# quziyan/NPairLoss

Measured on NVIDIA H100. Metric: N-pair fwd+bwd samples/sec at B=8192,D=512, higher is better.
Workload: dtype f32 (3-pass fp16-split wgmma, f32 accumulate)

## Files before the change

### npairloss_b200/csrc/ctx.cu

```cuda
#include <cuda.h>
#include <cuda_bf16.h>
#include <cuda_fp16.h>
#include <cuda_runtime.h>
#include <sched.h>
#include <cudaTypedefs.h>
#include <dlfcn.h>

#include <cstdarg>
#include <cstdio>
#include <cstdlib>
#include <cmath>
#include <cstring>
#include <map>
#include <memory>
#include <mutex>
#include <string>
#include <vector>

#include "../../include/npair_b200.h"
#include "gemm_wgmma.cuh"
#include "grad_fused.cuh"
#include "host.cuh"
#include "kernels.cuh"

// ... 436 lines not shown
  if (c->ev_made) for (int i = 0; i < NPAIR_PROF_PHASES; ++i) { cudaEventDestroy(c->ev[i][0]); cudaEventDestroy(c->ev[i][1]); }
  delete c;
}

static int create_impl(const npair_config* cfg, const void* id128, void* ext_comm, npair_ctx** out);
static bool mma_is_symmetric(int prec, int device) {
  static std::mutex mu;
  static std::map<std::pair<int, int>, bool> cache;
  std::lock_guard<std::mutex> lk(mu);
  const std::pair<int, int> key(device, prec);
  auto it = cache.find(key);
  if (it != cache.end()) return it->second;
  bool ok = false;
  const int Q = 192, D = 96;
  npair_config cfg;
  npair_config_default(&cfg, Q, D);
  cfg.sim_precision = prec; cfg.device = device; cfg.flags = NPAIR_INTERNAL_FULL_TILES; cfg.num_tops = 2;
  npair_ctx* t = nullptr;
  if (create_impl(&cfg, nullptr, nullptr, &t) == NPAIR_OK) {
    std::vector<float> x(static_cast<size_t>(Q) * D), lab(Q), S(static_cast<size_t>(Q) * t->ldS);
    uint32_t rng = 12345u;
    for (int r = 0; r < Q; ++r) {
      double nrm = 0.0;
      for (int d = 0; d < D; ++d) { rng = rng * 1664525u + 1013904223u; const float v = static_cast<float>(static_cast<int32_t>(rng >> 8) % 2001 - 1000) * 1e-3f; x[static_cast<size_t>(r) * D + d] = v; nrm += static_cast<double>(v) * v; }
      const float inv = static_cast<float>(1.0 / sqrt(nrm > 0 ? nrm : 1.0));
      for (int d = 0; d < D; ++d) x[static_cast<size_t>(r) * D + d] *= inv;
      lab[r] = static_cast<float>(r / 2);
    }
    float *dx = nullptr, *dl = nullptr;
    float tops[5];
    if (cudaMalloc(&dx, sizeof(float) * x.size()) == cudaSuccess && cudaMalloc(&dl, sizeof(float) * Q) == cudaSuccess &&
        cudaMemcpy(dx, x.data(), sizeof(float) * x.size(), cudaMemcpyHostToDevice) == cudaSuccess &&
        cudaMemcpy(dl, lab.data(), sizeof(float) * Q, cudaMemcpyHostToDevice) == cudaSuccess &&
        npair_forward(t, dx, dl, tops, nullptr) == NPAIR_OK && cudaDeviceSynchronize() == cudaSuccess &&
        cudaMemcpy(S.data(), t->S, sizeof(float) * S.size(), cudaMemcpyDeviceToHost) == cudaSuccess) {
      ok = true;
      for (int i = 0; i < Q && ok; ++i)
        for (int j = 0; j < i; ++j)
          if (memcmp(&S[static_cast<size_t>(i) * t->ldS + j], &S[static_cast<size_t>(j) * t->ldS + i], 4) != 0) { ok = false; break; }
    }
    cudaFree(dx); cudaFree(dl);
    npair_destroy(t);
  }
  cudaGetLastError();
  cache[key] = ok;
  return ok;
}

static int create_impl(const npair_config* cfg, const void* id128, void* ext_comm, npair_ctx** out) {
  if (!out) { g_create_err = "null out"; return NPAIR_E_ARG; }
  *out = nullptr;
  std::string e;
  int rc = validate(cfg, &e);
  if (rc != NPAIR_OK) { g_create_err = e; return rc; }
  int device = -1, sms = 0;
  if ((rc = open_device(cfg->device, &device, &sms)) != NPAIR_OK) return rc;
  std::unique_ptr<npair_ctx, void (*)(npair_ctx*)> made(new npair_ctx(), npair_destroy);
  npair_ctx* c = made.get();
  c->cfg = *cfg; c->device = device; c->sms = sms;
  const bool blocks = sim_block_rows(*cfg) > 0;
  const bool ask_sym = (cfg->world > 1 && cfg->bwd_exchange == NPAIR_BWD_AUTO && cfg->gemm_backend == NPAIR_GEMM_TCGEN05) || blocks;
  const bool sym = !ask_sym || mma_is_symmetric(cfg->sim_precision, c->device);
  if (blocks && !sym) {
    g_create_err = "row-block similarity mode: the similarity GEMM is not bitwise symmetric on this device, so a recomputed block of S "
                   "would not match the rows the statistics were taken from";
    return NPAIR_E_ARG;
  }
  static_cast<Plan&>(*c) = plan_of(*cfg, c->sms, sym);
  c->Q = cfg->Q; c->D = cfg->D; c->world = cfg->world; c->rank = cfg->rank; c->prec = cfg->sim_precision;
  const int Q = c->Q, D = c->D, N = c->N, ns = c->nsplit;
  CREATE_TRY(ctx_buffers(c, c->mem));
  if (c->sym_tiles) {
    const std::vector<int2> tl = sym_tile_list(Q, N);
    CREATE_TRY(cudaMemcpy(c->sym_tiles, tl.data(), sizeof(int2) * tl.size(), cudaMemcpyHostToDevice));
  }
  CREATE_TRY(cudaHostAlloc(&c->tops_pinned, sizeof(TopsBlock), cudaHostAllocMapped));
  memset(c->tops_pinned, 0, sizeof(TopsBlock));
  CREATE_TRY(cudaHostGetDevicePointer(&c->tops_dev, c->tops_pinned, 0));
  CREATE_TRY(c->order.create());
  if (c->lsel_mask) CREATE_TRY(allow_local_select_smem());
  if (cfg->gemm_backend == NPAIR_GEMM_TCGEN05) {
    CREATE_TRY(allow_smem(gemm_kernel(c->prec, c->sweep_epi)));
    if (c->n_blocks > 1) CREATE_TRY(allow_smem(gemm_kernel(c->prec, EPI_STORE_S)));
    CREATE_TRY(c->fused_grad ? allow_smem(fused_kernel(c->prec)) : allow_smem(gemm_kernel(c->prec, EPI_OUT)));
    std::string te;
    const int bkg = c->bk_grad;
    const uint16_t* catA = c->cat ? c->XcatA : c->Xs;
    const uint16_t* catB = c->cat ? c->XcatB : c->Xs;
    bool ok = make_tmap_kcat(&c->tm_simA, &c->tm_simB, catA +static_cast<long long>(c->rank) * Q * c->kcat, Q, catB, N, c->kcat, &te);
    ok = ok && make_tmap_f32_store(&c->tm_S, c->S, N, c->s_rows, c->ldS, &te);
    if (c->H) ok = ok && make_tmap_pieces(&c->tm_b1A, c->H, N, Q, ns, c->Np, static_cast<long long>(Q) * c->Np, bkg, 128, &te);
    ok = ok && make_tmap_pieces(&c->tm_b1B, c->XsT, N, D, ns, c->Np, static_cast<long long>(D) * c->Np, bkg, 256, &te);
    if (c->fused_grad) {
      ok = ok && make_tmap_pieces(&c->tm_fB, c->XsT, N, D, ns, c->Np, static_cast<long long>(D) * c->Np, 32, 256, &te);
      ok = ok && make_tmap_f32_store(&c->tm_fS, c->S, N, c->s_rows, c->ldS, &te, 128);
    }
    if (c->bwd_mode == NPAIR_BWDMODE_REDUCE_SCATTER) {
      ok = ok && make_tmap_pieces(&c->tm_b2A, c->HT, Q, N, ns, c->Qp, static_cast<long long>(N) * c->Qp, bkg, 128, &te);
      ok = ok && make_tmap_pieces(&c->tm_b2B, c->XlT, Q, D, ns, c->Qp, static_cast<long long>(D) * c->Qp, bkg, 256, &te);
    }
    if (!ok) { g_create_err = te; return NPAIR_E_CUDA; }
  }
  if (c->world > 1 && (id128 || ext_comm)) {
    NcclApi* api = nccl_api();
    if (!api->h || !api->err.empty()) { g_create_err = api->err; return NPAIR_E_NCCL; }
    if (ext_comm) { c->comm = ext_comm; c->own_comm = false; }
    else {
      std::string ce;
      if (acquire_comm(id128, c->world, c->rank, &c->comm, &ce) != 0) { g_create_err = ce; c->comm = nullptr; return NPAIR_E_NCCL; }
      c->own_comm = true;
    }
  }
  if (c->comm && (c->want_p2p_feat || c->want_p2p_rec) && !getenv("NPAIR_NO_P2P")) {
    NcclApi* api = nccl_api();
    const int W = c->world;
    CREATE_TRY(p2p_buffers(c, c->mem));
    cudaIpcMemHandle_t mine;
    static_assert(sizeof(cudaIpcMemHandle_t) == 64, "IPC handle size");
    CREATE_TRY(cudaIpcGetMemHandle(&mine, c->p2p_region));
    char* d_all = nullptr;
    CREATE_TRY(cudaMalloc(&d_all, 64ull * (W + 1)));
    const std::unique_ptr<char, cudaError_t (*)(void*)> free_handles(d_all, cudaFree);
    char* d_mine = d_all + 64ull * W;
    CREATE_TRY(cudaMemcpy(d_mine, &mine, 64, cudaMemcpyHostToDevice));
    CREATE_TRY(cudaDeviceSynchronize());
    int r = api->AllGather(d_mine, d_all, 16, NCCL_FLOAT32, c->comm, nullptr);
    if (r != 0) { g_create_err = fmt("ncclAllGather(ipc handles): %s", api->GetErrorString(r)); return NPAIR_E_NCCL; }
    CREATE_TRY(cudaStreamSynchronize(nullptr));
    std::vector<cudaIpcMemHandle_t> all(W);
    CREATE_TRY(cudaMemcpy(all.data(), d_all, 64ull * W, cudaMemcpyDeviceToHost));
    std::vector<float*> pb(W);
    bool mapped = true;
    for (int q = 0; q < W && mapped; ++q) {
      if (q == c->rank) { pb[q] = c->p2p_region; continue; }
      void* a = nullptr;
      if (cudaIpcOpenMemHandle(&a, all[q], cudaIpcMemLazyEnablePeerAccess) != cudaSuccess) { cudaGetLastError(); mapped = false; break; }
      c->p2p_opened.push_back(a);
      pb[q] = static_cast<float*>(a);
    }
    if (mapped) {
      CREATE_TRY(cudaMemcpy(c->p2p_peer_base, pb.data(), sizeof(float*) * W, cudaMemcpyHostToDevice));
      c->p2p_feat = c->want_p2p_feat; c->p2p_rec = c->want_p2p_rec;
    }
  }
  if (c->wscope && !c->comm) {
    g_create_err = "global_scope with world > 1 needs a communicator (the world-scope reductions are internal)"; return NPAIR_E_ARG;
  }
  *out = made.release();
  return NPAIR_OK;
}

int npair_create(const npair_config* cfg, const void* id128, npair_ctx** out) { return create_impl(cfg, id128, nullptr, out); }
int npair_create_with_comm(const npair_config* cfg, void* comm, npair_ctx** out) {
  if (cfg && cfg->world > 1 && !comm) { g_create_err = "null communicator"; return NPAIR_E_ARG; }
  return create_impl(cfg, nullptr, comm, out);
}

static void p2p_push(npair_ctx* c, int kind, uint32_t ep, int blocks, const float* srcA, long long nA, int partA,
                     const float* srcB, long long nB, int partB, cudaStream_t st) {
  const long long par = ep & 1u;
  p2p_push_kernel<<<blocks, 256, 0, st>>>(srcA, nA, c->xl.off(partA, par, c->rank), srcB, nB, srcB ? c->xl.off(partB, par, c->rank) : 0,
                                          c->p2p_peer_base, c->xl.flags, xchg_flag(kind, par, c->world, c->rank), c->world, ep, c->p2p_ticket);
  count_launch();
}
static const float* p2p_wait(npair_ctx* c, int kind, uint32_t ep, int part, cudaStream_t st) {
  const long long par = ep & 1u;
  p2p_wait_kernel<<<1, 32, 0, st>>>(reinterpret_cast<const uint32_t*>(c->p2p_region + c->xl.flags) + xchg_flag(kind, par, c->world, 0), c->world, ep);
// ... 247 lines not shown
  if (!c) return NPAIR_E_ARG;
  if (!d_feat || !d_label || !d_diff || !tops_host) { c->err = "null pointer argument"; return NPAIR_E_ARG; }
  int rc;
  if ((rc = check_out_aligned(c, d_diff, "the gradient pointer")) != NPAIR_OK) return rc;
  if ((rc = need_comm(c, "npair_forward_gathered")) != NPAIR_OK) return rc;
  OrderedCall call(c, stream);
  if ((rc = call.enter()) != NPAIR_OK) return rc;
  if ((rc = forward_rank(c, d_feat, d_label, call.st)) != NPAIR_OK) return rc;
  if ((rc = backward_impl(c, loss_weight, d_diff, nullptr, nullptr, call.st)) != NPAIR_OK) return rc;
  return finish_forward(c, tops_host, call.st);
}

int npair_backward_partial(npair_ctx* c, float loss_weight, float* d_local_half, float* d_total_half, void* stream) {
  if (!c) return NPAIR_E_ARG;
  if (!d_local_half || (c->world > 1 && !d_total_half)) { c->err = "null gradient pointer"; return NPAIR_E_ARG; }
  int rc;
  if ((rc = check_out_aligned(c, d_local_half, "d_local_half")) != NPAIR_OK) return rc;
  if (c->world > 1 && (rc = check_out_aligned(c, d_total_half, "d_total_half")) != NPAIR_OK) return rc;
  if ((rc = need_forward(c, "npair_backward_partial")) != NPAIR_OK) return rc;
  if (c->bwd_mode == NPAIR_BWDMODE_ROW_SCALARS) { c->err = "this context exchanges row scalars: use npair_row_scalars + npair_backward_gathered"; return NPAIR_E_STATE; }
  OrderedCall call(c, stream);
  if ((rc = call.enter()) != NPAIR_OK) return rc;
  return backward_impl(c, loss_weight, d_local_half, c->world > 1 ? d_total_half : nullptr, nullptr, call.st);
}

int npair_row_scalars(npair_ctx* c, float* d_out, void* stream) {
  if (!c || !d_out) return NPAIR_E_ARG;
  int rc;
  if ((rc = need_forward(c, "npair_row_scalars")) != NPAIR_OK) return rc;
  OrderedCall call(c, stream);
  if ((rc = call.enter()) != NPAIR_OK) return rc;
  CUDA_TRY(c, cudaMemcpyAsync(d_out, c->ra.rowrec, sizeof(RowRecord) * c->Q, cudaMemcpyDeviceToDevice, call.st));
  return NPAIR_OK;
}

int npair_backward_gathered(npair_ctx* c, float loss_weight, const float* d_rs_total, float* d_diff, void* stream) {
  if (!c) return NPAIR_E_ARG;
  if (!d_rs_total || !d_diff) { c->err = "null pointer argument"; return NPAIR_E_ARG; }
  int rc;
  if ((rc = check_out_aligned(c, d_diff, "the gradient pointer")) != NPAIR_OK) return rc;
  if ((rc = need_forward(c, "npair_backward_gathered")) != NPAIR_OK) return rc;
  if (c->bwd_mode != NPAIR_BWDMODE_ROW_SCALARS) { c->err = "this context does not exchange row scalars (see npair_bwd_exchange_mode)"; return NPAIR_E_STATE; }
  OrderedCall call(c, stream);
  if ((rc = call.enter()) != NPAIR_OK) return rc;
  return backward_impl(c, loss_weight, d_diff, nullptr, reinterpret_cast<const RowRecord*>(d_rs_total), call.st);
}

static void reduce_splits(npair_ctx* c, int splits, int rows, float* d_diff, float beta, cudaStream_t st) {
  const long long n = split_part(1, rows, c->D);
  splitk_reduce_kernel<<<grid_for(n / 4, 8 * c->sms), 256, 0, st>>>(c->part, splits, n, d_diff, beta);
  count_launch();
}

static int backward_core(npair_ctx* c, float loss_weight, float* d_diff, float* d_total_ext, const RowRecord* d_rs_ext, cudaStream_t st) {
  const int Q = c->Q, N = c->N, D = c->D;
  const MiningParams mp = mining_of(c->cfg);
  const float lw_over_q = loss_weight / static_cast<float>(c->wscope ? N : Q);
  const bool tc = c->cfg.gemm_backend == NPAIR_GEMM_TCGEN05;
  const RowRecord* rs_total = nullptr;
  int bw_mode = BW_SYM;
  if (c->bwd_mode == NPAIR_BWDMODE_ROW_SCALARS) {
    bw_mode = BW_ROWSCAL;
    if (d_rs_ext) rs_total = d_rs_ext;
    else {
      if (c->p2p_rec && !c->step.ext_gathered) {
        PhaseTimer pt(c, 8, st);
        rs_total = reinterpret_cast<const RowRecord*>(p2p_wait(c, XCHG_RECORDS, c->p2p_rec_epoch, XP_REC, st));
      } else if (!c->step.rec_gathered) {
        PhaseTimer pt(c, 8, st);
        NcclApi* api = nccl_api();
        int r = api->AllGather(c->ra.rowrec, c->rs_total, ROW_RECORD_FLOATS * Q, NCCL_FLOAT32, c->comm, st);
        if (r != 0) { c->err = fmt("ncclAllGather(row records): %s", api->GetErrorString(r)); return NPAIR_E_NCCL; }
        c->step.rec_gathered = true;
        rs_total = c->rs_total;
      } else rs_total = c->rs_total;
    }
  } else if (c->bwd_mode == NPAIR_BWDMODE_REDUCE_SCATTER) bw_mode = BW_SPLIT;
  if (tc && c->fused_grad) {
    FusedGradParams fp; memset(&fp, 0, sizeof(fp));
    fp.N = N; fp.D = D;
    fp.colrec = rs_total ? rs_total : c->ra.rowrec;
    fp.inv_world = c->wscope ? 1.f : 1.f / static_cast<float>(c->world);
    fp.log2_world = c->wscope ? 0.f : log2f(static_cast<float>(c->world));
    fp.sgn_p = ap_sign(mp.ap_method); fp.sgn_n = an_sign(mp.an_method);
    fp.ldo = D; fp.alpha = 0.5f * lw_over_q; fp.beta = 0.f; fp.dev_scale = &c->bs->x_inv_scale;
    fp.part = c->part;
    fp.chunk_kb = c->grad_chunk_kb;
    PhaseTimer pt(c, 6, st);
    const int first = c->s_block_row0 >= 0 ? c->s_block_row0 / c->s_rows : 0;
    for (int k = 0; k < c->n_blocks; ++k) {
      const int r0 = (first + k) % c->n_blocks * c->s_rows, rows = Q - r0 < c->s_rows ? Q - r0 : c->s_rows;
      CUDA_TRY(c, recompute_sim_block(c, r0, st));
      const SimRows sim = sim_rows(c, r0, rows);
      fp.Q = sim.rows; fp.ts = tile_sched(sim.rows, D, c->grad_kblocks, c->grad_split); fp.m_blk0 = sim.row0 / TileShape::BM;
      fp.rowrec = c->ra.rowrec + sim.row0; fp.self_offset = sim.self_col(sim.row0); fp.out = d_diff + static_cast<long long>(sim.row0) * D;
      CUDA_TRY(c, launch_fused_grad(c->prec, c->tm_fB, c->tm_fS, fp, c->sms, st));
      if (fp.ts.splits > 1) reduce_splits(c, fp.ts.splits, rows, fp.out, 0.f, st);
    }
    CUDA_TRY(c, cudaGetLastError());
    return NPAIR_OK;
  }
  {
    PhaseTimer pt(c, 5, st);
    launch_build_weights(sim_rows(c, 0, Q), c->world, bw_mode, rs_total, mp, c->ra, c->prec, c->H, c->Np, c->HT, c->Qp, st);
  }
  GemmParams gp; memset(&gp, 0, sizeof(gp));
  gp.dev_scale = &c->bs->x_inv_scale;
  const bool rs_path = c->bwd_mode == NPAIR_BWDMODE_REDUCE_SCATTER;
  if (rs_path) {
    gp.M = N; gp.Nn = D; gp.ts = tile_sched(N, D, (Q + c->bk_grad - 1) / c->bk_grad);
    gp.out = d_total_ext ? d_total_ext : c->OUT2; gp.ldo = D; gp.alpha = 0.5f * (1.f / static_cast<float>(c->world)) * lw_over_q; gp.beta = 0.f;
    {
      PhaseTimer pt(c, 7, st);
      if (tc) CUDA_TRY(c, launch_gemm(c->prec, EPI_OUT,c->tm_b2A, c->tm_b2B, c->tm_S, gp, c->sms, st));
      else CUDA_TRY(c, launch_simt_gemm(c->prec, EPI_OUT, c->HT, c->Qp, static_cast<long long>(N) * c->Qp, c->XlT, c->Qp, static_cast<long long>(D) * c->Qp, Q, gp, st));
    }
    if (!d_total_ext) {
      PhaseTimer pt(c, 8, st);
      NcclApi* api = nccl_api();
      int r = api->ReduceScatter(c->OUT2, d_diff, static_cast<size_t>(Q) * D, NCCL_FLOAT32, NCCL_SUM, c->comm, st);
      if (r != 0) { c->err = fmt("ncclReduceScatter: %s", api->GetErrorString(r)); return NPAIR_E_NCCL; }
    }
  }
  gp.M = Q; gp.Nn = D; gp.ts = tile_sched(Q, D, c->grad_kblocks, c->grad_split);
  gp.out = d_diff; gp.ldo = D; gp.alpha = 0.5f * lw_over_q; gp.beta = (rs_path && !d_total_ext) ? 1.f : 0.f;
  gp.part = c->part;
  {
    PhaseTimer pt(c, 6, st);
    if (tc) CUDA_TRY(c, launch_gemm(c->prec, EPI_OUT,c->tm_b1A, c->tm_b1B, c->tm_S, gp, c->sms, st));
    else CUDA_TRY(c, launch_simt_gemm(c->prec, EPI_OUT, c->H, c->Np, static_cast<long long>(Q) * c->Np, c->XsT, c->Np, static_cast<long long>(D) * c->Np, N, gp, st));
    if (gp.ts.splits > 1) reduce_splits(c, gp.ts.splits, Q, d_diff, gp.beta, st);
  }
  CUDA_TRY(c, cudaGetLastError());
  return NPAIR_OK;
}

int npair_profile_enable(npair_ctx* c, int on) {
  if (!c) return NPAIR_E_ARG;
  CUDA_TRY(c, cudaSetDevice(c->device));
  if (on && !c->ev_made) {
    for (int i = 0; i < NPAIR_PROF_PHASES; ++i) { CUDA_TRY(c, cudaEventCreate(&c->ev[i][0])); CUDA_TRY(c, cudaEventCreate(&c->ev[i][1])); }
    c->ev_made = true;
  }
  c->prof = on != 0;
  for (int i = 0; i < NPAIR_PROF_PHASES; ++i) c->ev_used[i] = false;
  return NPAIR_OK;
}
unsigned long long npair_kernel_launches(void) { return npair::g_kernel_launches; }

static int await_calls(npair_ctx* c) {
  CUDA_TRY(c, cudaSetDevice(c->device));
  CUDA_TRY(c, cudaEventSynchronize(c->order.done));
  return NPAIR_OK;
}

int npair_profile_read(npair_ctx* c, float* ms_out) {
  if (!c || !ms_out) return NPAIR_E_ARG;
  const int rc = await_calls(c);
  if (rc != NPAIR_OK) return rc;
  for (int i = 0; i < NPAIR_PROF_PHASES; ++i) {
    ms_out[i] = 0.f;
    if (c->ev_made && c->ev_used[i]) { float ms = 0.f; CUDA_TRY(c, cudaEventElapsedTime(&ms, c->ev[i][0], c->ev[i][1])); ms_out[i] = ms; }
    c->ev_used[i] = false;
  }
  return NPAIR_OK;
}

__global__ void decode_ord_kernel(const uint32_t* __restrict__ in, float* __restrict__ out, int n) {
  const int i = blockIdx.x * blockDim.x + threadIdx.x;
  if (i < n) out[i] = ord2f(in[i]);
}
__global__ void int_to_float_kernel(const int* __restrict__ in, float* __restrict__ out, int n) {
  const int i = blockIdx.x * blockDim.x + threadIdx.x;
  if (i < n) out[i] = static_cast<float>(in[i]);
}

int npair_debug_read(npair_ctx* c, int which, float* dst, size_t n) {
  if (!c || !dst) return NPAIR_E_ARG;
  const int rc = await_calls(c);
// ... 131 lines not shown
```

### npairloss_b200/csrc/gemm.cu

```cuda
#include <cuda_bf16.h>
#include <cuda_fp16.h>
#include <cuda_runtime.h>

#include "gemm_wgmma.cuh"
#include "grad_fused.cuh"
#include "host.cuh"
#include "kernels.cuh"

namespace npair {

static int gemm_grid(const TileSched& ts, int sms) { return ts.num_tiles() < sms ? ts.num_tiles() : sms; }

template <int NSPLIT, bool BF16, int EPI, int BK>
static GemmKernel gemm_t() {
  using Cfg = GemmCfg<NSPLIT, BK, EPI>;
  return GemmKernel{split_gemm_kernel<NSPLIT, BF16, EPI, BK>, Cfg::THREADS, Cfg::SMEM_BYTES};
}
template <bool BF16>
static GemmKernel sim_gemm_t(int epi) {
  switch (epi) {
    case EPI_STORE_S | EPI_STATS: return gemm_t<1, BF16, EPI_STORE_S | EPI_STATS, 64>();
    case EPI_STORE_S | EPI_STATS | EPI_SYM: return gemm_t<1, BF16, EPI_STORE_S | EPI_STATS | EPI_SYM, 64>();
    case EPI_STATS: return gemm_t<1, BF16, EPI_STATS, 64>();
    case EPI_STATS | EPI_SYM: return gemm_t<1, BF16, EPI_STATS | EPI_SYM, 64>();
    case EPI_STORE_S: return gemm_t<1, BF16, EPI_STORE_S, 64>();
    case EPI_COUNT: return gemm_t<1, BF16, EPI_COUNT, 64>();
    case EPI_COUNT | EPI_SYM: return gemm_t<1, BF16, EPI_COUNT | EPI_SYM, 64>();
    case EPI_GATHER: return gemm_t<1, BF16, EPI_GATHER, 64>();
    case EPI_GATHER | EPI_SYM: return gemm_t<1, BF16, EPI_GATHER | EPI_SYM, 64>();
    case EPI_BUCKET: return gemm_t<1, BF16, EPI_BUCKET, 64>();
    case EPI_BUCKET | EPI_SYM: return gemm_t<1, BF16, EPI_BUCKET | EPI_SYM, 64>();
    case EPI_ARGMAX: return gemm_t<1, BF16, EPI_ARGMAX, 64>();
    default: return GemmKernel{nullptr, 0, 0};
  }
}
GemmKernel gemm_kernel(int prec, int epi) {
  return with_prec(prec, [epi](auto P) {
    constexpr SplitFormat f = SPLIT_FORMATS[P];
    return epi != EPI_OUT ? sim_gemm_t<f.bf16>(epi) : gemm_t<f.pieces, f.bf16, EPI_OUT, bk_of(P, EPI_OUT)>();
  });
}
cudaError_t launch_gemm(int prec, int epi, const CUtensorMap& a, const CUtensorMap& b, const CUtensorMap& sm, const GemmParams& p, int sms, cudaStream_t st) {
  const GemmKernel k = gemm_kernel(prec, epi);
  if (!k.fn) return cudaErrorInvalidValue;
  k.fn<<<gemm_grid(p.ts, sms), k.threads, k.smem, st>>>(a, b, sm, p);
  count_launch();
  return cudaGetLastError();
}

FusedKernel fused_kernel(int prec) {
  return with_prec(prec, [](auto P) {
    constexpr SplitFormat f = SPLIT_FORMATS[P];
    return FusedKernel{fused_grad_kernel<f.pieces, f.bf16>, FusedCfg<f.pieces>::THREADS, FusedCfg<f.pieces>::SMEM_BYTES};
  });
}
cudaError_t launch_fused_grad(int prec, const CUtensorMap& b, const CUtensorMap& sm, const FusedGradParams& p, int sms, cudaStream_t st) {
  const FusedKernel k = fused_kernel(prec);
  k.fn<<<gemm_grid(p.ts, sms), k.threads, k.smem, st>>>(b, sm, p);
  count_launch();
  return cudaGetLastError();
}

template <int PREC>
__device__ __forceinline__ float piece_sum(const uint16_t* base, long long off, long long ps) {
  if (PREC == PREC_BF16) return __bfloat162float(__ushort_as_bfloat16(base[off]));
  if (PREC == PREC_FP16X2) return __half2float(__ushort_as_half(base[off])) + __half2float(__ushort_as_half(base[ps + off]));
  return __bfloat162float(__ushort_as_bfloat16(base[off])) + __bfloat162float(__ushort_as_bfloat16(base[ps + off])) +
         __bfloat162float(__ushort_as_bfloat16(base[2 * ps + off]));
}
template <int PREC, int OUT>
__global__ void __launch_bounds__(256) simt_gemm_kernel(const uint16_t* __restrict__ A, long long lda, long long psA,
                                                        const uint16_t* __restrict__ B, long long ldb, long long psB, int K, GemmParams p) {
  __shared__ float As[16][65], Bs[16][65];
  const int tx = threadIdx.x & 15, ty = threadIdx.x >> 4;
  const int m0 = blockIdx.y * 64, n0 = blockIdx.x * 64;
  float acc[4][4] = {};
  for (int k0 = 0; k0 < K; k0 += 16) {
    for (int e = threadIdx.x; e < 64 * 16; e += 256) {
      const int r = e >> 4, kk = e & 15;
      const int gm = m0 + r, gn = n0 + r, gk = k0 + kk;
      As[kk][r] = (gm < p.M && gk < K) ? piece_sum<PREC>(A, static_cast<long long>(gm) * lda + gk, psA) : 0.f;
      Bs[kk][r] = (gn < p.Nn && gk < K) ? piece_sum<PREC>(B, static_cast<long long>(gn) * ldb + gk, psB) : 0.f;
    }
    __syncthreads();
#pragma unroll
    for (int kk = 0; kk < 16; ++kk) {
      float a[4], b[4];
#pragma unroll
      for (int i = 0; i < 4; ++i) { a[i] = As[kk][ty * 4 + i]; b[i] = Bs[kk][tx * 4 + i]; }
#pragma unroll
      for (int i = 0; i < 4; ++i)
#pragma unroll
        for (int j = 0; j < 4; ++j) acc[i][j] = fmaf(a[i], b[j], acc[i][j]);
    }
    __syncthreads();
  }
  const float inv = p.dev_scale ? *p.dev_scale : 1.f;
  for (int i = 0; i < 4; ++i) {
    const int row = m0 + ty * 4 + i;
    if (row >= p.M) continue;
    for (int j = 0; j < 4; ++j) {
      const int col = n0 + tx * 4 + j;
      if (col >= p.Nn) continue;
      if (!OUT) p.S[static_cast<long long>(row) * p.ldS + col] = acc[i][j] * inv * inv;
      else {
        float* d = p.out + static_cast<long long>(row) * p.ldo + col;
        float o = p.alpha * inv * acc[i][j];
        if (p.beta != 0.f) o += p.beta * *d;
        *d = o;
      }
    }
  }
}
cudaError_t launch_simt_gemm(int prec, int epi, const uint16_t* A, long long lda, long long psA, const uint16_t* B, long long ldb,
                             long long psB, int K, const GemmParams& p, cudaStream_t st) {
  dim3 grid((p.Nn + 63) / 64, (p.M + 63) / 64);
  with_prec(prec, [&](auto P) {
    auto kernel = epi == EPI_OUT ? simt_gemm_kernel<P, 1> : simt_gemm_kernel<P, 0>;
    kernel<<<grid, 256, 0, st>>>(A, lda, psA, B, ldb, psB, K, p);
  });
  count_launch();
  return cudaGetLastError();
}

__global__ void splitk_reduce_kernel(const float* __restrict__ part, int splits, long long n, float* __restrict__ out, float beta) {
  const long long t0 = static_cast<long long>(blockIdx.x) * blockDim.x + threadIdx.x, nth = static_cast<long long>(gridDim.x) * blockDim.x;
  const bool vec = (n & 3) == 0 && ((reinterpret_cast<uintptr_t>(part) | reinterpret_cast<uintptr_t>(out)) & 15) == 0;
  if (vec) {
    for (long long i = t0 * 4; i < n; i += nth * 4) {
      float4 a = *reinterpret_cast<const float4*>(part + i);
      for (int s = 1; s < splits; ++s) { const float4 b = *reinterpret_cast<const float4*>(part + s * n + i); a.x += b.x; a.y += b.y; a.z += b.z; a.w += b.w; }
      if (beta != 0.f) { const float4 o = *reinterpret_cast<const float4*>(out + i); a.x += beta * o.x; a.y += beta * o.y; a.z += beta * o.z; a.w += beta * o.w; }
      *reinterpret_cast<float4*>(out + i) = a;
    }
  } else {
    for (long long i = t0; i < n; i += nth) {
      float a = part[i];
      for (int s = 1; s < splits; ++s) a += part[s * n + i];
      if (beta != 0.f) a += beta * out[i];
      out[i] = a;
// ... 6 lines not shown
```

### npairloss_b200/csrc/grad_fused.cuh

```cuda
#pragma once
#include <cuda.h>
#include <cuda_bf16.h>
#include <cuda_fp16.h>
#include <cuda_runtime.h>
#include <stdint.h>

#include "gemm_wgmma.cuh"
#include "ptx.cuh"

namespace npair {

struct FusedGradParams {
  int Q, N, D;
  TileSched ts;
  int chunk_kb;
  float* part;
  const float* S;
  const RowRecord* rowrec;
  const RowRecord* colrec;
  int self_offset;
  float inv_world, log2_world;
  float sgn_p, sgn_n;
  float* out; long long ldo;
  float alpha, beta;
  const float* dev_scale;
  int m_blk0;
};

template <int NSPLIT>
struct FusedCfg {
  static constexpr int BM = 128, BN = 256, BK = 32;
  static constexpr int B_PIECE = BN * 64;
  static constexpr int S_TILE = BM * 128;
  static constexpr int CREC = BK * sizeof(RowRecord);
  static constexpr int STAGE_BYTES = NSPLIT * B_PIECE + S_TILE + CREC;
  static constexpr int NPASS = mma_passes(NSPLIT);
  static constexpr int STAGES_FIT = (227 * 1024 - 2048) / STAGE_BYTES;
  static constexpr int STAGES = STAGES_FIT > 6 ? 6 : STAGES_FIT;
  static constexpr int SMEM_BYTES = STAGES * STAGE_BYTES + 1024  + 1024 ;
  static constexpr int THREADS = 384;
};

template <int NSPLIT, bool BF16>
__device__ __forceinline__ void split_pair(float a, float b, uint32_t (&out)[3]) {
  if (NSPLIT == 1) {
    out[0] = static_cast<uint32_t>(__bfloat16_as_ushort(__float2bfloat16_rn(a))) | (static_cast<uint32_t>(__bfloat16_as_ushort(__float2bfloat16_rn(b))) << 16);
  } else if (NSPLIT == 2) {
    const __half2 h = __floats2half2_rn(a, b);
    const float2 hf = __half22float2(h);
    const __half2 l = __floats2half2_rn(a - hf.x, b - hf.y);
    out[0] = *reinterpret_cast<const uint32_t*>(&h);
    out[1] = *reinterpret_cast<const uint32_t*>(&l);
  } else {
    const __nv_bfloat162 h = __floats2bfloat162_rn(a, b);
    const float2 hf = __bfloat1622float2(h);
    const float r1a = a - hf.x, r1b = b - hf.y;
    const __nv_bfloat162 m = __floats2bfloat162_rn(r1a, r1b);
    const float2 mf = __bfloat1622float2(m);
    const __nv_bfloat162 l = __floats2bfloat162_rn(r1a - mf.x, r1b - mf.y);
    out[0] = *reinterpret_cast<const uint32_t*>(&h);
    out[1] = *reinterpret_cast<const uint32_t*>(&m);
    out[2] = *reinterpret_cast<const uint32_t*>(&l);
  }
}

__device__ __forceinline__ void red_add_v2(float* dst, float a, float b) {
  asm volatile("red.global.add.v2.f32 [%0], {%1, %2};" ::"l"(dst), "f"(a), "f"(b) : "memory");
}
__device__ __forceinline__ void red_add_f32(float* dst, float a) {
  asm volatile("red.global.add.f32 [%0], %1;" ::"l"(dst), "f"(a) : "memory");
}

__device__ __forceinline__ void bulk_copy_g2s(void* smem_dst, const void* gsrc, uint32_t bytes, uint64_t* bar) {
  asm volatile("cp.async.bulk.shared::cluster.global.mbarrier::complete_tx::bytes [%0], [%1], %2, [%3];"
               ::"r"(ptx::smem_u32(smem_dst)), "l"(reinterpret_cast<uint64_t>(gsrc)), "r"(bytes), "r"(ptx::smem_u32(bar))
               : "memory");
}

__device__ __forceinline__ int chunk_end(int c0, int kb0, int kb1, int ch, int key) {
  if (ch <= 0) return kb1;
  if (c0 == kb0) { const int first = max(1, (((key & 7) + 1) * ch) >> 3); return min(kb1, kb0 + first); }
  return min(kb1, c0 + ch);
}

struct RowRec { float m2r, tn, m2, lab, tp, cA; int self_col; };

__device__ __forceinline__ float select_f32(bool c, float a, float b) {
  float r;
  asm("{\n\t.reg .pred q;\n\tsetp.ne.b32 q, %3, 0;\n\tselp.f32 %0, %1, %2, q;\n\t}" : "=f"(r) : "f"(a), "f"(b), "r"(static_cast<int>(c)));
  return r;
}
__device__ __forceinline__ float pair_weight(float s, const RowRecord& c, const RowRec& r, int m, const FusedGradParams& p) {
  const bool same = !(c.label() != r.lab);
  const float kn = s * p.sgn_n;
  const float a1 = select_f32(same, fmaf(s, LOG2E, -r.m2), select_f32(kn <= r.tn, fmaf(s, LOG2E, -r.m2r), -INFINITY));
  const float a2 = select_f32(same, fmaf(s, LOG2E, -c.m2()), select_f32(kn <= c.thr_n(), fmaf(s, LOG2E, -c.m2c()), -INFINITY));
  float e1, e2;
  asm("ex2.approx.ftz.f32 %0, %1;" : "=f"(e1) : "f"(a1));
  asm("ex2.approx.ftz.f32 %0, %1;" : "=f"(e2) : "f"(a2));
  const float kp = s * p.sgn_p;
  const float w1 = select_f32(kp <= r.tp, e1 * r.cA, 0.f);
  const float w2 = select_f32(kp <= c.thr_p(), e2 * c.cA(), 0.f);
  const float g = select_f32(same, fmaf(w2, p.inv_world, w1), e1 + e2);
  return (m == r.self_col || m >= p.N) ? 0.f : g;
}

__device__ __forceinline__ RowRec load_rowrec(const FusedGradParams& p, int row) {
  RowRec r;
  r.m2 = 0.f; r.m2r = INFINITY; r.tp = -INFINITY; r.tn = -INFINITY; r.cA = 0.f; r.lab = 0.f;
  r.self_col = row + p.self_offset;
  if (row < p.Q) {
    const RowRecord c = p.rowrec[row];
    r.m2r = c.m2c() - p.log2_world; r.tn = c.thr_n(); r.m2 = c.m2(); r.lab = c.label(); r.tp = c.thr_p(); r.cA = c.cA();
  }
  return r;
}

template <int NSPLIT, bool BF16>
__global__ void __launch_bounds__(384, 1)
fused_grad_kernel(const __grid_constant__ CUtensorMap tmapB, const __grid_constant__ CUtensorMap tmapS, const FusedGradParams p) {
  using Cfg = FusedCfg<NSPLIT>;
  const int worker = static_cast<int>(blockIdx.x), num_workers = static_cast<int>(gridDim.x);
  constexpr int BM = Cfg::BM, BN = Cfg::BN, BK = Cfg::BK, STAGES = Cfg::STAGES;
  extern __shared__ uint8_t smem_raw[];
  uint8_t* smem = smem_raw + ((1024u - (ptx::smem_u32(smem_raw) & 1023u)) & 1023u);
  StageRing<STAGES> ring(smem + STAGES * Cfg::STAGE_BYTES);

  const int warp = threadIdx.x >> 5, lane = threadIdx.x & 31;
  const int num_tiles = p.ts.num_tiles();
  const float inv_scale = p.dev_scale ? *p.dev_scale : 1.f;
  const float alpha = p.alpha * inv_scale;

  if (warp == 8 && lane == 0) {
    ptx::prefetch_tmap(&tmapB); ptx::prefetch_tmap(&tmapS);
    ring.init();
  }
  __syncthreads();

  if (warp >= 8) {
    asm volatile("setmaxnreg.dec.sync.aligned.u32 40;");
    if (warp == 8 && lane == 0) {
      for (int tile = worker; tile < num_tiles; tile += num_workers) {
        const Tile t = p.ts.at(tile);
        for (int kb = t.kb0; kb < t.kb1; ++kb) {
          const int m0 = kb * BK;
          const uint32_t crec_bytes = static_cast<uint32_t>(min(BK, p.N - m0)) * static_cast<uint32_t>(sizeof(RowRecord));
          uint64_t* full = ring.produce(NSPLIT * Cfg::B_PIECE + Cfg::S_TILE + crec_bytes);
          uint8_t* st = smem + ring.stage * Cfg::STAGE_BYTES;
#pragma unroll
          for (int s = 0; s < NSPLIT; ++s)
            ptx::tma_load_3d(st + s * Cfg::B_PIECE, &tmapB, full, m0, t.n_blk * BN, s);
          ptx::tma_load_2d(st + NSPLIT * Cfg::B_PIECE, &tmapS, full, m0, t.m_blk * BM);
          bulk_copy_g2s(st + NSPLIT * Cfg::B_PIECE + Cfg::S_TILE, p.colrec + m0, crec_bytes, full);
          ring.advance();
        }
      }
    }
  } else {
    asm volatile("setmaxnreg.inc.sync.aligned.u32 232;");
    constexpr int KSTEPS = BK / 16;
    static_assert(KSTEPS % 2 == 0, "a K block's first step must use A buffer 0");
    const int g = warp >> 2, wi = warp & 3;
    const int c4 = lane & 3;
    const int rl0 = g * 64 + wi * 16 + (lane >> 2);
    auto build = [&](uint32_t (&af)[NSPLIT][4], const RowRec (&rr)[2], int st_idx, int kb, int k2) {
      const uint8_t* s_tile = smem + st_idx * Cfg::STAGE_BYTES + NSPLIT * Cfg::B_PIECE;
      const RowRecord* crec = reinterpret_cast<const RowRecord*>(s_tile + Cfg::S_TILE);
#pragma unroll
      for (int t = 0; t < 2; ++t) {
        const int k = 16 * k2 + 8 * t + 2 * c4;
        const int m = kb * BK + k;
        const RowRecord c0 = RowRecord::load(crec, k), c1 = RowRecord::load(crec, k + 1);
#pragma unroll
        for (int h = 0; h < 2; ++h) {
          const int rl = rl0 + 8 * h;
          const float2 s2 = *reinterpret_cast<const float2*>(s_tile + rl * 128 + (((k >> 2) ^ (rl & 7)) << 4) + (k & 3) * 4);
          const float w0 = pair_weight(s2.x, c0, rr[h], m, p);
          const float w1 = pair_weight(s2.y, c1, rr[h], m + 1, p);
          uint32_t o[3];
          split_pair<NSPLIT, BF16>(w0, w1, o);
#pragma unroll
          for (int s = 0; s < NSPLIT; ++s) af[s][2 * t + h] = o[s];
        }
      }
    };
    for (int tile = worker; tile < num_tiles; tile += num_workers) {
      const Tile t = p.ts.at(tile);
      const int ckey = ((p.m_blk0 + t.m_blk) >> 1) + t.n_blk + t.split;
      float* obase = p.ts.splits > 1 ? p.part + split_part(t.split, p.Q, p.ldo) : p.out;
      const float beta = p.ts.splits > 1 ? 0.f : p.beta;
      RowRec rr[2];
#pragma unroll
      for (int h = 0; h < 2; ++h) rr[h] = load_rowrec(p, t.m_blk * BM + rl0 + 8 * h);
      float acc[128];
      uint32_t af[2][NSPLIT][4];
      for (int c0 = t.kb0, c1; c0 < t.kb1; c0 = c1) {
        c1 = chunk_end(c0, t.kb0, t.kb1, p.chunk_kb, ckey);
        ring.wait_full();
        build(af[0], rr, ring.stage, c0, 0);
        int prev = ring.stage;
        for (int kb = c0; kb < c1; ++kb) {
          const int cur = ring.stage;
          const uint32_t b0 = ptx::smem_u32(smem + cur * Cfg::STAGE_BYTES);
          ring.advance();
#pragma unroll
          for (int k2 = 0; k2 < KSTEPS; ++k2) {
            ptx::wgmma_fence();
#pragma unroll
            for (int ps = 0; ps < Cfg::NPASS; ++ps) {
              int sa, sb;
              pass_pieces(NSPLIT, ps, sa, sb);
              const uint64_t bd = ptx::make_kmajor_desc(b0 + sb * Cfg::B_PIECE + k2 * 32, 512u, 2u);
              ptx::wgmma_m64n256k16_rs<BF16>(acc, af[k2 & 1][sa], bd, ((kb - c0) | ps | k2) != 0 ? 1u : 0u);
            }
            ptx::wgmma_commit();
            ptx::wgmma_wait<1>();
            if (k2 == 0 && kb != c0) ring.release(prev, lane);
            if (k2 + 1 < KSTEPS) {
              build(af[(k2 + 1) & 1], rr, cur, kb, k2 + 1);
            } else if (kb + 1 < c1) {
              ring.wait_full();
              build(af[0], rr, ring.stage, kb + 1, 0);
            }
          }
          prev = cur;
        }
        ptx::wgmma_wait<0>();
        ptx::fence_regs(acc);
        ring.release(prev, lane);
        const bool first = (c0 == t.kb0);
#pragma unroll
        for (int j = 0; j < 32; ++j) {
          const int col = t.n_blk * BN + 8 * j + 2 * c4;
#pragma unroll
          for (int h = 0; h < 2; ++h) {
            const int row = t.m_blk * BM + rl0 + 8 * h;
            if (row >= p.Q || col >= p.D) continue;
            float* dst = obase + static_cast<long long>(row) * p.ldo + col;
            float o0 = alpha * acc[4 * j + 2 * h], o1 = alpha * acc[4 * j + 2 * h + 1];
            if (col + 1 < p.D && (p.ldo & 1) == 0) {
              if (first) {
                if (beta != 0.f) { const float2 old = *reinterpret_cast<const float2*>(dst); o0 += beta * old.x; o1 += beta * old.y; }
                *reinterpret_cast<float2*>(dst) = make_float2(o0, o1);
              } else red_add_v2(dst, o0, o1);
            } else {
              if (first) dst[0] = (beta != 0.f) ? o0 + beta * dst[0] : o0; else red_add_f32(dst, o0);
              if (col + 1 < p.D) { if (first) dst[1] = (beta != 0.f) ? o1 + beta * dst[1] : o1; else red_add_f32(dst + 1, o1); }
            }
          }
        }
      }
    }
  }
}

}
```

### npairloss_b200/csrc/host.cuh

```cuda
#pragma once
#include <cuda.h>
#include <cuda_runtime.h>

#include <cstdarg>
#include <cstdio>
#include <cstring>
#include <string>
#include <vector>

#include "../../include/npair_b200.h"
#include "gemm_wgmma.cuh"
#include "grad_fused.cuh"
#include "kernels.cuh"

namespace npair {

extern thread_local std::string g_create_err;

inline std::string fmt(const char* f, ...) {
  char buf[1024];
  va_list ap; va_start(ap, f); vsnprintf(buf, sizeof(buf), f, ap); va_end(ap);
  return std::string(buf);
}

bool make_tmap_pieces(CUtensorMap* m, const void* base, int cols, int rows, int pieces, long long ld_elems, long long piece_stride_elems,
                      int bk, int box_rows, std::string* err);
bool make_tmap_kcat(CUtensorMap* a, CUtensorMap* b, const uint16_t* A, int rows_a, const uint16_t* B, int rows_b, long long kcat,
                    std::string* err);
bool make_tmap_f32_store(CUtensorMap* m, const void* base, int cols, int rows, long long ld_elems, std::string* err, int box_rows = 32);

constexpr int bk_of(int prec, int epi) {
  if (epi != EPI_OUT) return 64;
  return prec == PREC_BF16 ? 64 : 32;
}

struct GemmKernel { void (*fn)(CUtensorMap, CUtensorMap, CUtensorMap, GemmParams); int threads, smem; };
struct FusedKernel { void (*fn)(CUtensorMap, CUtensorMap, FusedGradParams); int threads, smem; };
template <class K>
cudaError_t allow_smem(const K& k) {
  return k.fn ? cudaFuncSetAttribute(k.fn, cudaFuncAttributeMaxDynamicSharedMemorySize, k.smem) : cudaErrorInvalidValue;
}
GemmKernel gemm_kernel(int prec, int epi);
cudaError_t launch_gemm(int prec, int epi, const CUtensorMap& a, const CUtensorMap& b, const CUtensorMap& sm, const GemmParams& p, int sms, cudaStream_t st);
FusedKernel fused_kernel(int prec);
cudaError_t launch_fused_grad(int prec, const CUtensorMap& b, const CUtensorMap& sm, const FusedGradParams& p, int sms, cudaStream_t st);
cudaError_t launch_simt_gemm(int prec, int epi, const uint16_t* A, long long lda, long long psA, const uint16_t* B, long long ldb,
                             long long psB, int K, const GemmParams& p, cudaStream_t st);
__global__ void splitk_reduce_kernel(const float* __restrict__ part, int splits, long long n, float* __restrict__ out, float beta);

struct SplitK { int splits, kb_per_split; };
inline SplitK split_k(int num_kblocks, int tiles, int sms, int min_kb) {
  int splits = sms / (tiles > 0 ? tiles : 1);
  if (splits > 16) splits = 16;
  if (splits > num_kblocks / min_kb) splits = num_kblocks / min_kb;
  if (splits < 1) splits = 1;
  const int kpb = (num_kblocks + splits - 1) / splits;
  return SplitK{(num_kblocks + kpb - 1) / kpb, kpb};
}

using TileShape = GemmCfg<1, 64, EPI_OUT>;
static_assert(TileShape::BM == FusedCfg<1>::BM && TileShape::BN == FusedCfg<1>::BN, "both GEMM kernels share one tile shape");
inline TileSched tile_sched(int rows, int cols, int num_kblocks, SplitK sk) {
  return TileSched{num_kblocks, (rows + TileShape::BM - 1) / TileShape::BM, (cols + TileShape::BN - 1) / TileShape::BN, nullptr, 0, sk.splits, sk.kb_per_split};
}
inline TileSched tile_sched(int rows, int cols, int num_kblocks) { return tile_sched(rows, cols, num_kblocks, SplitK{1, num_kblocks}); }

inline int grid_for(long long work, int max_blocks) {
  const long long nb = (work + 255) / 256;
  return static_cast<int>(nb < 1 ? 1 : (nb > max_blocks ? max_blocks : nb));
}

inline long long round_up(long long v, long long m) { return (v + m - 1) / m * m; }

inline std::vector<int2> sym_tile_list(int Q, int N) {
  std::vector<int2> tl;
  const TileSched ts = tile_sched(Q, N, 0);
  for (int mb = 0; mb < ts.tiles_m; ++mb)
    for (int nb = mb / 2; nb < ts.tiles_n; ++nb) tl.push_back(make_int2(mb, nb));
  return tl;
}
inline long long sym_tile_count(int Q, int N) {
  const TileSched ts = tile_sched(Q, N, 0);
  long long n = 0;
  for (int mb = 0; mb < ts.tiles_m; ++mb) n += mb / 2 < ts.tiles_n ? ts.tiles_n - mb / 2 : 0;
  return n;
}

inline GemmParams sim_sweep(int epi, int rows, int cols, long long kcat, const float* inv_scale, const int2* sym_tiles, int n_sym_tiles,
                            const RowArrays& ra) {
  GemmParams gp; memset(&gp, 0, sizeof(gp));
  gp.M = rows; gp.Nn = cols;
  gp.ts = tile_sched(rows, cols, static_cast<int>(kcat / 64));
  gp.dev_scale = inv_scale;
  if (epi & EPI_SYM) { gp.ts.tile_list = sym_tiles; gp.ts.num_tiles_list = n_sym_tiles; }
  if (epi & EPI_STATS) {
    gp.st_minw = ra.st_minw; gp.st_maxw = ra.st_maxw; gp.st_maxb = ra.st_maxb; gp.st_maxall = ra.st_maxall; gp.cnt_same = ra.cnt_same;
  }
  return gp;
}

struct Carve {
  char* base;
  size_t bytes = 0;
  template <class T>
  T* take(long long count, size_t align = alignof(T)) {
    bytes = (bytes + align - 1) / align * align;
    T* p = base ? reinterpret_cast<T*>(base + bytes) : nullptr;
    bytes += sizeof(T) * count;
    return p;
  }
};

struct DevMem {
  explicit DevMem(bool allocate = true) : allocate(allocate) {}
  DevMem(const DevMem&) = delete;
  ~DevMem() { release(); }
  template <class T>
  void own(T** p, size_t n, bool zero) {
    if (n == 0 || err != cudaSuccess) return;
    bytes += n;
    if (!allocate) return;
    if ((err = cudaMalloc(p, n)) != cudaSuccess) { *p = nullptr; return; }
    held.push_back(*p);
    if (zero) err = cudaMemset(*p, 0, n);
  }
  template <class F>
  void own_carved(bool zero, F carve) {
    Carve size{nullptr}, cut{nullptr};
// ... 72 lines not shown
```

Before: 10.18 million.

## Specialize fused grad kernel on signs, skip masking, overlap weight compute with wgmma

Turns the positive and negative sign factors into template parameters, giving four kernel instantiations chosen on the host. It also simplifies the pair-weight select logic and drops the self/bounds mask on k-blocks that cannot contain the diagonal or the tail. Weight computation for the next k-step now runs right after issuing the first-pass wgmma, before the wait, while packing into fp16 pieces stays after the wait. The aim is to hide SIMT exp work behind tensor-core execution and cut ALU work, at the cost of more instantiations and higher register pressure.

```diff
diff --git a/npairloss_b200/csrc/ctx.cu b/npairloss_b200/csrc/ctx.cu
--- a/npairloss_b200/csrc/ctx.cu
+++ b/npairloss_b200/csrc/ctx.cu
@@ -542,7 +542,7 @@
   if (cfg->gemm_backend == NPAIR_GEMM_TCGEN05) {
     CREATE_TRY(allow_smem(gemm_kernel(c->prec, c->sweep_epi)));
     if (c->n_blocks > 1) CREATE_TRY(allow_smem(gemm_kernel(c->prec, EPI_STORE_S)));
-    CREATE_TRY(c->fused_grad ? allow_smem(fused_kernel(c->prec)) : allow_smem(gemm_kernel(c->prec, EPI_OUT)));
+    CREATE_TRY(c->fused_grad ? allow_smem(fused_kernel(c->prec, cfg->ap_method, cfg->an_method)) : allow_smem(gemm_kernel(c->prec, EPI_OUT)));
     std::string te;
     const int bkg = c->bk_grad;
     const uint16_t* catA = c->cat ? c->XcatA : c->Xs;
@@ -956,7 +956,6 @@
     fp.colrec = rs_total ? rs_total : c->ra.rowrec;
     fp.inv_world = c->wscope ? 1.f : 1.f / static_cast<float>(c->world);
     fp.log2_world = c->wscope ? 0.f : log2f(static_cast<float>(c->world));
-    fp.sgn_p = ap_sign(mp.ap_method); fp.sgn_n = an_sign(mp.an_method);
     fp.ldo = D; fp.alpha = 0.5f * lw_over_q; fp.beta = 0.f; fp.dev_scale = &c->bs->x_inv_scale;
     fp.part = c->part;
     fp.chunk_kb = c->grad_chunk_kb;
@@ -968,7 +967,7 @@
       const SimRows sim = sim_rows(c, r0, rows);
       fp.Q = sim.rows; fp.ts = tile_sched(sim.rows, D, c->grad_kblocks, c->grad_split); fp.m_blk0 = sim.row0 / TileShape::BM;
       fp.rowrec = c->ra.rowrec + sim.row0; fp.self_offset = sim.self_col(sim.row0); fp.out = d_diff + static_cast<long long>(sim.row0) * D;
-      CUDA_TRY(c, launch_fused_grad(c->prec, c->tm_fB, c->tm_fS, fp, c->sms, st));
+      CUDA_TRY(c, launch_fused_grad(c->prec, mp.ap_method, mp.an_method, c->tm_fB, c->tm_fS, fp, c->sms, st));
       if (fp.ts.splits > 1) reduce_splits(c, fp.ts.splits, rows, fp.out, 0.f, st);
     }
     CUDA_TRY(c, cudaGetLastError());
diff --git a/npairloss_b200/csrc/gemm.cu b/npairloss_b200/csrc/gemm.cu
--- a/npairloss_b200/csrc/gemm.cu
+++ b/npairloss_b200/csrc/gemm.cu
@@ -48,14 +48,22 @@
   return cudaGetLastError();
 }
 
-FusedKernel fused_kernel(int prec) {
-  return with_prec(prec, [](auto P) {
+template <int NSPLIT, bool BF16>
+static FusedKernel fused_t(bool neg_p, bool neg_n) {
+  auto fn = neg_p ? (neg_n ? fused_grad_kernel<NSPLIT, BF16, true, true> : fused_grad_kernel<NSPLIT, BF16, true, false>)
+                  : (neg_n ? fused_grad_kernel<NSPLIT, BF16, false, true> : fused_grad_kernel<NSPLIT, BF16, false, false>);
+  return FusedKernel{fn, FusedCfg<NSPLIT>::THREADS, FusedCfg<NSPLIT>::SMEM_BYTES};
+}
+FusedKernel fused_kernel(int prec, int ap_method, int an_method) {
+  const bool neg_p = ap_sign(ap_method) < 0.f, neg_n = an_sign(an_method) < 0.f;
+  return with_prec(prec, [=](auto P) {
     constexpr SplitFormat f = SPLIT_FORMATS[P];
-    return FusedKernel{fused_grad_kernel<f.pieces, f.bf16>, FusedCfg<f.pieces>::THREADS, FusedCfg<f.pieces>::SMEM_BYTES};
+    return fused_t<f.pieces, f.bf16>(neg_p, neg_n);
   });
 }
-cudaError_t launch_fused_grad(int prec, const CUtensorMap& b, const CUtensorMap& sm, const FusedGradParams& p, int sms, cudaStream_t st) {
-  const FusedKernel k = fused_kernel(prec);
+cudaError_t launch_fused_grad(int prec, int ap_method, int an_method, const CUtensorMap& b, const CUtensorMap& sm, const FusedGradParams& p,
+                              int sms, cudaStream_t st) {
+  const FusedKernel k = fused_kernel(prec, ap_method, an_method);
   k.fn<<<gemm_grid(p.ts, sms), k.threads, k.smem, st>>>(b, sm, p);
   count_launch();
   return cudaGetLastError();
diff --git a/npairloss_b200/csrc/grad_fused.cuh b/npairloss_b200/csrc/grad_fused.cuh
--- a/npairloss_b200/csrc/grad_fused.cuh
+++ b/npairloss_b200/csrc/grad_fused.cuh
@@ -4,6 +4,8 @@
 #include <cuda_fp16.h>
 #include <cuda_runtime.h>
 #include <stdint.h>
+
+#include <type_traits>
 
 #include "gemm_wgmma.cuh"
 #include "ptx.cuh"
@@ -20,7 +22,6 @@
   const RowRecord* colrec;
   int self_offset;
   float inv_world, log2_world;
-  float sgn_p, sgn_n;
   float* out; long long ldo;
   float alpha, beta;
   const float* dev_scale;
@@ -90,19 +91,20 @@
   asm("{\n\t.reg .pred q;\n\tsetp.ne.b32 q, %3, 0;\n\tselp.f32 %0, %1, %2, q;\n\t}" : "=f"(r) : "f"(a), "f"(b), "r"(static_cast<int>(c)));
   return r;
 }
+template <bool NEG_P, bool NEG_N, bool MASK>
 __device__ __forceinline__ float pair_weight(float s, const RowRecord& c, const RowRec& r, int m, const FusedGradParams& p) {
   const bool same = !(c.label() != r.lab);
-  const float kn = s * p.sgn_n;
-  const float a1 = select_f32(same, fmaf(s, LOG2E, -r.m2), select_f32(kn <= r.tn, fmaf(s, LOG2E, -r.m2r), -INFINITY));
-  const float a2 = select_f32(same, fmaf(s, LOG2E, -c.m2()), select_f32(kn <= c.thr_n(), fmaf(s, LOG2E, -c.m2c()), -INFINITY));
+  const float k = NEG_P == NEG_N ? (NEG_P ? -s : s) : select_f32(same, NEG_P ? -s : s, NEG_N ? -s : s);
+  const bool ok1 = k <= select_f32(same, r.tp, r.tn), ok2 = k <= select_f32(same, c.thr_p(), c.thr_n());
+  const float a1 = select_f32(ok1, fmaf(s, LOG2E, -select_f32(same, r.m2, r.m2r)), -INFINITY);
+  const float a2 = select_f32(ok2, fmaf(s, LOG2E, -select_f32(same, c.m2(), c.m2c())), -INFINITY);
   float e1, e2;
   asm("ex2.approx.ftz.f32 %0, %1;" : "=f"(e1) : "f"(a1));
   asm("ex2.approx.ftz.f32 %0, %1;" : "=f"(e2) : "f"(a2));
-  const float kp = s * p.sgn_p;
-  const float w1 = select_f32(kp <= r.tp, e1 * r.cA, 0.f);
-  const float w2 = select_f32(kp <= c.thr_p(), e2 * c.cA(), 0.f);
+  const float w1 = e1 * select_f32(ok1, r.cA, 0.f);
+  const float w2 = e2 * select_f32(ok2, c.cA(), 0.f);
   const float g = select_f32(same, fmaf(w2, p.inv_world, w1), e1 + e2);
-  return (m == r.self_col || m >= p.N) ? 0.f : g;
+  return MASK && (m == r.self_col || m >= p.N) ? 0.f : g;
 }
 
 __device__ __forceinline__ RowRec load_rowrec(const FusedGradParams& p, int row) {
@@ -116,7 +118,7 @@
   return r;
 }
 
-template <int NSPLIT, bool BF16>
+template <int NSPLIT, bool BF16, bool NEG_P, bool NEG_N>
 __global__ void __launch_bounds__(384, 1)
 fused_grad_kernel(const __grid_constant__ CUtensorMap tmapB, const __grid_constant__ CUtensorMap tmapS, const FusedGradParams p) {
   using Cfg = FusedCfg<NSPLIT>;
@@ -163,7 +165,7 @@
     const int g = warp >> 2, wi = warp & 3;
     const int c4 = lane & 3;
     const int rl0 = g * 64 + wi * 16 + (lane >> 2);
-    auto build = [&](uint32_t (&af)[NSPLIT][4], const RowRec (&rr)[2], int st_idx, int kb, int k2) {
+    auto weights_as = [&](auto masked, float (&w)[8], const RowRec (&rr)[2], int st_idx, int kb, int k2) {
       const uint8_t* s_tile = smem + st_idx * Cfg::STAGE_BYTES + NSPLIT * Cfg::B_PIECE;
       const RowRecord* crec = reinterpret_cast<const RowRecord*>(s_tile + Cfg::S_TILE);
 #pragma unroll
@@ -175,13 +177,22 @@
         for (int h = 0; h < 2; ++h) {
           const int rl = rl0 + 8 * h;
           const float2 s2 = *reinterpret_cast<const float2*>(s_tile + rl * 128 + (((k >> 2) ^ (rl & 7)) << 4) + (k & 3) * 4);
-          const float w0 = pair_weight(s2.x, c0, rr[h], m, p);
-          const float w1 = pair_weight(s2.y, c1, rr[h], m + 1, p);
-          uint32_t o[3];
-          split_pair<NSPLIT, BF16>(w0, w1, o);
-#pragma unroll
-          for (int s = 0; s < NSPLIT; ++s) af[s][2 * t + h] = o[s];
-        }
+          w[4 * t + 2 * h] = pair_weight<NEG_P, NEG_N, decltype(masked)::value>(s2.x, c0, rr[h], m, p);
+          w[4 * t + 2 * h + 1] = pair_weight<NEG_P, NEG_N, decltype(masked)::value>(s2.y, c1, rr[h], m + 1, p);
+        }
+      }
+    };
+    auto weights = [&](bool masked, float (&w)[8], const RowRec (&rr)[2], int st_idx, int kb, int k2) {
+      if (masked) weights_as(std::true_type{}, w, rr, st_idx, kb, k2);
+      else weights_as(std::false_type{}, w, rr, st_idx, kb, k2);
+    };
+    auto pack = [&](uint32_t (&af)[NSPLIT][4], const float (&w)[8]) {
+#pragma unroll
+      for (int i = 0; i < 4; ++i) {
+        uint32_t o[3];
+        split_pair<NSPLIT, BF16>(w[2 * i], w[2 * i + 1], o);
+#pragma unroll
+        for (int s = 0; s < NSPLIT; ++s) af[s][i] = o[s];
       }
     };
     for (int tile = worker; tile < num_tiles; tile += num_workers) {
@@ -192,12 +203,17 @@
       RowRec rr[2];
 #pragma unroll
       for (int h = 0; h < 2; ++h) rr[h] = load_rowrec(p, t.m_blk * BM + rl0 + 8 * h);
+      const int self0 = t.m_blk * BM + p.self_offset;
+      auto masked_kb = [&](int kb) { const int m0 = kb * BK; return (m0 < self0 + BM && m0 + BK > self0) || m0 + BK > p.N; };
       float acc[128];
       uint32_t af[2][NSPLIT][4];
       for (int c0 = t.kb0, c1; c0 < t.kb1; c0 = c1) {
         c1 = chunk_end(c0, t.kb0, t.kb1, p.chunk_kb, ckey);
         ring.wait_full();
-        build(af[0], rr, ring.stage, c0, 0);
+        bool mk = masked_kb(c0);
+        float w[8];
+        weights(mk, w, rr, ring.stage, c0, 0);
+        pack(af[0], w);
         int prev = ring.stage;
         for (int kb = c0; kb < c1; ++kb) {
           const int cur = ring.stage;
@@ -212,16 +228,21 @@
               pass_pieces(NSPLIT, ps, sa, sb);
               const uint64_t bd = ptx::make_kmajor_desc(b0 + sb * Cfg::B_PIECE + k2 * 32, 512u, 2u);
               ptx::wgmma_m64n256k16_rs<BF16>(acc, af[k2 & 1][sa], bd, ((kb - c0) | ps | k2) != 0 ? 1u : 0u);
+              if (ps == 0) {
+                if (k2 + 1 < KSTEPS) {
+                  weights(mk, w, rr, cur, kb, k2 + 1);
+                } else if (kb + 1 < c1) {
+                  ring.wait_full();
+                  mk = masked_kb(kb + 1);
+                  weights(mk, w, rr, ring.stage, kb + 1, 0);
+                }
+              }
             }
             ptx::wgmma_commit();
+            const bool next = k2 + 1 < KSTEPS || kb + 1 < c1;
             ptx::wgmma_wait<1>();
             if (k2 == 0 && kb != c0) ring.release(prev, lane);
-            if (k2 + 1 < KSTEPS) {
-              build(af[(k2 + 1) & 1], rr, cur, kb, k2 + 1);
-            } else if (kb + 1 < c1) {
-              ring.wait_full();
-              build(af[0], rr, ring.stage, kb + 1, 0);
-            }
+            if (next) pack(af[(k2 + 1) & 1], w);
           }
           prev = cur;
         }
diff --git a/npairloss_b200/csrc/host.cuh b/npairloss_b200/csrc/host.cuh
--- a/npairloss_b200/csrc/host.cuh
+++ b/npairloss_b200/csrc/host.cuh
@@ -42,8 +42,9 @@
 }
 GemmKernel gemm_kernel(int prec, int epi);
 cudaError_t launch_gemm(int prec, int epi, const CUtensorMap& a, const CUtensorMap& b, const CUtensorMap& sm, const GemmParams& p, int sms, cudaStream_t st);
-FusedKernel fused_kernel(int prec);
-cudaError_t launch_fused_grad(int prec, const CUtensorMap& b, const CUtensorMap& sm, const FusedGradParams& p, int sms, cudaStream_t st);
+FusedKernel fused_kernel(int prec, int ap_method, int an_method);
+cudaError_t launch_fused_grad(int prec, int ap_method, int an_method, const CUtensorMap& b, const CUtensorMap& sm, const FusedGradParams& p,
+                              int sms, cudaStream_t st);
 cudaError_t launch_simt_gemm(int prec, int epi, const uint16_t* A, long long lda, long long psA, const uint16_t* B, long long ldb,
                              long long psB, int K, const GemmParams& p, cudaStream_t st);
 __global__ void splitk_reduce_kernel(const float* __restrict__ part, int splits, long long n, float* __restrict__ out, float beta);
```

Result: faster. 10.54 million, median of 6 (+3.6%).
